# lewisjiang/contour-context

Hardware: AMD Instinct MI355X
Metric: scans/sec ingest+query (120k-pt scan vs 5k-scan DB); max-F1 parity (higher is better)
Workload: dtype f32+f64

## Files before the change

### contour-context_amd/csrc/cc_db_api.inc

```

namespace {

#define CC_ZC_MAX 64
#define CC_NVIEW 4
#define CC_NSTAGE 4
struct ScanLite {
  float keys[CC_NQLEV][CC_NPIV][CC_KEY_DIM];
  int n_cont[CC_HOT_LEVELS];
  int flags;
};

}

#define CC_N_HEADS 24
__global__ void __launch_bounds__(256)
cc_k_pack_hot(const cc_scan_desc_t *__restrict__ desc, int n, cc_hot_desc_t *__restrict__ hot,
              int *__restrict__ z_heads , int *__restrict__ z_pass_cnt ,
              const cc_query_meta *__restrict__ meta_src ,
              cc_query_meta *__restrict__ meta_dst, const int *__restrict__ sel ) {
  const int i = blockIdx.x;
  if (i >= n) return;
  const cc_scan_desc_t *d = desc + (sel ? sel[i] : i);
  cc_hot_desc_t *o = hot + i;
  const int tid = threadIdx.x, nt = blockDim.x;
// ... 486 lines not shown
  if (!db || n < 1 || n > cc_db::NLANE) return set_err(CC_EINVAL, "cc_db_set_lanes: 1 .. 4 lanes");
  {
    const int rc = cc_db_query_wait(db);
    if (rc != CC_OK) return rc;
  }
  HIPCHK(hipSetDevice(db->device));
  for (int i = 0; i < n; i++) {
    const int rc = lane_alloc(db, db->lane[i]);
    if (rc != CC_OK) return rc;
  }
  db->n_lanes = n;
  db->next_lane = 0;
  return CC_OK;
}

int cc_db_size(const cc_db *db) { return db ? db->n_scans : 0; }
int cc_db_knn_stride(const cc_db *db) { return db ? db->kmax : 0; }

void cc_packed_sizes(size_t *hot_bytes, size_t *feat_bytes) {
  if (hot_bytes) *hot_bytes = sizeof(cc_hot_desc_t);
  if (feat_bytes) *feat_bytes = sizeof(cc_gmm_feat);
}
const void *cc_db_hot_ptr(const cc_db *db) { return db ? db->d_hot : nullptr; }
const void *cc_db_feat_ptr(const cc_db *db) { return db ? db->d_feat : nullptr; }

int cc_db_bucket_state(const cc_db *db, int32_t *tree_sizes, float *ranges) {
  if (!db || !tree_sizes || !ranges) return set_err(CC_EINVAL, "cc_db_bucket_state: bad argument");
  for (int l = 0; l < CC_NQLEV; l++) {
    for (int b = 0; b < 6; b++) tree_sizes[l * 6 + b] = (l < db->cfg.n_q_levels) ? (int32_t)db->book[l].b[b].tree.size() : 0;
    for (int b = 0; b < 7; b++) ranges[l * 7 + b] = (l < db->cfg.n_q_levels) ? db->book[l].ranges[b] : 0.f;
  }
  return CC_OK;
}

#define DB_DRAIN(db)                            \
  {                                             \
    const int drc_ = cc_db_query_wait(db);      \
    if (drc_ != CC_OK) return drc_;             \
  }
#define DB_POISON_CHK(db, what) \
  if ((db)->poisoned) return set_err(CC_EHIP, what ": the database handle is in a failed state (an earlier HIP error); destroy it")

int cc_db_set_dynamic_thres(cc_db *db, int on) {
  if (!db || (on != 0 && on != 1)) return set_err(CC_EINVAL, "cc_db_set_dynamic_thres: db must be valid and on 0 or 1");
  DB_POISON_CHK(db, "cc_db_set_dynamic_thres");
  if (on) {
    HIPCHK(hipSetDevice(db->device));
    for (auto &ln : db->lane)
      if (ln.d_qmeta) {
        const int rc = lane_alloc_dyn(ln);
        if (rc != CC_OK) return rc;
      }
  }
  db->dyn_thres = on;
  return CC_OK;
}

static void push_idx_state(cc_db *db) {
  bool all = true;
  for (int l = 0; l < db->cfg.n_q_levels; l++) all = all && db->book[l].fullyIndexed();
  if (all) {
    db->idx_slot.push_back(-1);
    return;
  }
  cc_db::IdxRec r;
  for (int l = 0; l < CC_NQLEV; l++) {
    r.full[l] = (l >= db->cfg.n_q_levels || db->book[l].fullyIndexed()) ? 1 : 0;
    for (int b = 0; b < 6; b++) {
      r.iv[l][2 * b] = l < db->cfg.n_q_levels ? db->book[l].b[b].idx_lo : 0.f;
      r.iv[l][2 * b + 1] = l < db->cfg.n_q_levels ? db->book[l].b[b].idx_hi : 0.f;
    }
  }
  db->idx_slot.push_back((int)db->idx_store.size());
  db->idx_store.push_back(r);
}

int cc_pack_scans(cc_ctx *ctx, const cc_scan_desc_t *d_desc, int n, void *d_hot_out, void *d_feat_out, void *stream_) {
  if (!ctx || !d_desc || n < 0 || !d_hot_out || !d_feat_out) return set_err(CC_EINVAL, "cc_pack_scans: bad argument");
  if (n == 0) return CC_OK;
  hipStream_t stream = (hipStream_t)stream_;
  HIPCHK(hipSetDevice(ctx->device));
  hipLaunchKernelGGL(cc_k_pack_hot, dim3(n), dim3(256), 0, stream, d_desc, n, (cc_hot_desc_t *)d_hot_out, (int *)nullptr, (int *)nullptr,
                     (const cc_query_meta *)nullptr, (cc_query_meta *)nullptr, (const int *)nullptr);
  hipLaunchKernelGGL(cc_k_gmm_prep, dim3(n), dim3(CC_GMM_PREP_BLOCK), 0, stream, d_desc, n, (cc_gmm_feat *)d_feat_out, (const int *)nullptr);
  HIPCHK(hipGetLastError());
  return CC_OK;
}

static int fetch_lite(cc_db *db, const cc_hot_desc_t *d_hot, int n, ScanLite *h_out, hipStream_t stream) {
  if (n <= CC_ZC_MAX) {
    hipLaunchKernelGGL(cc_k_extract, dim3(n), dim3(64), 0, stream, d_hot, n, db->cfg.n_q_levels, db->cfg.q_levels[0], db->cfg.q_levels[1],
                       db->cfg.q_levels[2], db->h_lite_zc);
    HIPCHK(hipGetLastError());
    HIPCHK(hipStreamSynchronize(stream));
    memcpy(h_out, db->h_lite_zc, sizeof(ScanLite) * (size_t)n);
    return CC_OK;
  }
  for (int b0 = 0; b0 < n; b0 += 4096) {
    const int nb = n - b0 < 4096 ? n - b0 : 4096;
    hipLaunchKernelGGL(cc_k_extract, dim3(nb), dim3(64), 0, stream, d_hot + b0, nb, db->cfg.n_q_levels, db->cfg.q_levels[0],
                       db->cfg.q_levels[1], db->cfg.q_levels[2], db->d_lite);
    HIPCHK(hipGetLastError());
    HIPCHK(hipMemcpyAsync(h_out + b0, db->d_lite, sizeof(ScanLite) * nb, hipMemcpyDeviceToHost, stream));
    HIPCHK(hipStreamSynchronize(stream));
  }
  return CC_OK;
}

static int add_settle(cc_db *db) {
  if (db->add_pending) {
    db->add_pending = false;
    HIPCHK(hipEventSynchronize(db->add_done));
  }
  return CC_OK;
}

static int add_scans_device_part(cc_db *db, const int *old_n, const std::vector<int> *ent, const int *act_lo, hipStream_t stream) {
  const int nql = db->cfg.n_q_levels;
  if (db->add_done && db->add_stream != stream) HIPCHK(hipStreamWaitEvent(stream, db->add_done, 0));
  cc_kappend_params AP;
  size_t used = 0;
  size_t need = 0;
  for (int l = 0; l < nql; l++) need += ent[l].size() + (act_lo[l] < db->n_keys[l] ? (size_t)(db->n_keys[l] - act_lo[l]) : 0);
  if (need > db->add_cap) return set_err(CC_ECAPACITY, "cc_db_add_scans: staging buffer too small");
  const bool small_stage = need <= (size_t)CC_ZC_MAX * 64;
  int *h_stage = db->h_add;
  int stage_slot = -1;
  if (small_stage) {
    stage_slot = db->add_small_next;
    db->add_small_next = (stage_slot + 1) % CC_NSTAGE;
    if (db->add_small_busy[stage_slot]) {
      HIPCHK(hipEventSynchronize(db->add_small_ev[stage_slot]));
      db->add_small_busy[stage_slot] = false;
    }
    h_stage = db->h_add_small[stage_slot];
  } else {
    const int src_ = add_settle(db);
    if (src_ != CC_OK) return src_;
  }
  AP.cap_k = db->cap_k;
  for (int l = 0; l < CC_NQLEV; l++) {
    AP.keys[l] = db->d_keys[l];
    AP.kgidx[l] = db->d_kgidx[l];
    AP.kseq[l] = db->d_kseq[l];
    AP.n_old[l] = l < nql ? old_n[l] : 0;
    AP.q_levels[l] = l < nql ? db->cfg.q_levels[l] : 1;
    AP.first[l] = (int)used;
    if (l < nql && !ent[l].empty()) {
      memcpy(h_stage + used, ent[l].data(), sizeof(int) * ent[l].size());
      used += ent[l].size();
    }
  }
  AP.first[CC_NQLEV] = (int)used;
  const size_t n_ent = used;
  size_t act_off[CC_NQLEV] = {0, 0, 0};
  for (int l = 0; l < nql; l++) {
    act_off[l] = used;
    if (act_lo[l] < db->n_keys[l]) {
      const size_t cnt = (size_t)(db->n_keys[l] - act_lo[l]);
      memcpy(h_stage + used, db->book[l].active_from.data() + act_lo[l], sizeof(int) * cnt);
      used += cnt;
    }
  }
  const bool zc = used <= (size_t)CC_ZC_MAX * 64;
  size_t act_total = 0;
  for (int l = 0; l < CC_NQLEV; l++) {
    AP.act_first[l] = (int)act_total;
// ... 151 lines not shown
int cc_db_add_scans(cc_db *db, const cc_scan_desc_t *d_desc, int n, const double *h_ts, const int32_t *h_seed, void *stream_) {
  if (!db || !d_desc || n < 0 || !h_ts || !h_seed) return set_err(CC_EINVAL, "cc_db_add_scans: bad argument");
  DB_POISON_CHK(db, "cc_db_add_scans");
  if (db->n_scans + n > db->cap) return set_err(CC_ECAPACITY, "cc_db_add_scans: database capacity exceeded");
  if (n == 0) return CC_OK;
  hipStream_t stream = (hipStream_t)stream_;
  HIPCHK(hipSetDevice(db->device));
  if (db->prep_cnt > 0) {
    cc_db::Prepared &pp = db->prep[db->prep_head];
    if (pp.d_desc != d_desc || pp.n != n || pp.row0 != db->n_scans)
      return set_err(CC_EINVAL, "cc_db_add_scans: batches prepared with cc_db_add_scans_prepare must be added first, in the order they were prepared");
    HIPCHK(hipStreamWaitEvent(stream, pp.ev, 0));
    HIPCHK(hipEventSynchronize(pp.ev));
    db->prep_head = (db->prep_head + 1) % cc_db::PREP_SLOTS;
    db->prep_cnt--;
    db->n_prepared -= n;
    const int rc_p = add_scans_commit(db, n, h_ts, h_seed, stream, pp.h_lite);
    if (rc_p != CC_OK && db->prep_cnt > 0) {
      cc_db::Prepared &nx = db->prep[db->prep_head];
      hipEventSynchronize(nx.ev);
      db->prep_cnt = 0;
      db->n_prepared = 0;
    }
    return rc_p;
  }
  int rc = cc_pack_scans(db->ctx, d_desc, n, db->d_hot + db->n_scans, db->d_feat + db->n_scans, stream_);
  if (rc != CC_OK) return rc;
  return add_scans_commit(db, n, h_ts, h_seed, stream);
}

int cc_db_add_scans_prepare(cc_db *db, const cc_scan_desc_t *d_desc, int n, void *stream_) {
  if (!db || !d_desc || n < 1 || n > cc_db::PREP_MAX) return set_err(CC_EINVAL, "cc_db_add_scans_prepare: bad argument (1..4096 scans)");
  DB_POISON_CHK(db, "cc_db_add_scans_prepare");
  if (db->prep_cnt >= cc_db::PREP_SLOTS) return set_err(CC_EINVAL, "cc_db_add_scans_prepare: two prepared batches are already waiting to be added");
  if (db->n_scans + db->n_prepared + n > db->cap) return set_err(CC_ECAPACITY, "cc_db_add_scans_prepare: database capacity exceeded");
  hipStream_t stream = (hipStream_t)stream_;
  HIPCHK(hipSetDevice(db->device));
  cc_db::Prepared &pp = db->prep[(db->prep_head + db->prep_cnt) % cc_db::PREP_SLOTS];
  if (!pp.ev) {
    HIPCHK(hipEventCreateWithFlags(&pp.ev, hipEventDisableTiming));
    HIPCHK(hipMalloc(&pp.d_lite, sizeof(ScanLite) * cc_db::PREP_MAX));
    HIPCHK(hipHostMalloc((void **)&pp.h_lite, sizeof(ScanLite) * cc_db::PREP_MAX, hipHostMallocDefault));
  }
  const int row0 = db->n_scans + db->n_prepared;
  int rc = cc_pack_scans(db->ctx, d_desc, n, db->d_hot + row0, db->d_feat + row0, stream_);
  if (rc != CC_OK) return rc;
  hipLaunchKernelGGL(cc_k_extract, dim3(n), dim3(64), 0, stream, (const cc_hot_desc_t *)(db->d_hot + row0), n, db->cfg.n_q_levels,
                     db->cfg.q_levels[0], db->cfg.q_levels[1], db->cfg.q_levels[2], pp.d_lite);
  HIPCHK(hipGetLastError());
  HIPCHK(hipMemcpyAsync(pp.h_lite, pp.d_lite, sizeof(ScanLite) * (size_t)n, hipMemcpyDeviceToHost, stream));
  HIPCHK(hipEventRecord(pp.ev, stream));
  pp.d_desc = d_desc;
  pp.n = n;
  pp.row0 = row0;
  db->prep_cnt++;
  db->n_prepared += n;
  return CC_OK;
}

int cc_db_add_packed(cc_db *db, const void *d_hot, const void *d_feat, int n, const double *h_ts, const int32_t *h_seed, void *stream_) {
  if (!db || !d_hot || !d_feat || n < 0 || !h_ts || !h_seed) return set_err(CC_EINVAL, "cc_db_add_packed: bad argument");
  DB_POISON_CHK(db, "cc_db_add_packed");
  if (db->prep_cnt > 0) return set_err(CC_EINVAL, "cc_db_add_packed: batches prepared with cc_db_add_scans_prepare are waiting to be added");
  if (db->n_scans + n > db->cap) return set_err(CC_ECAPACITY, "cc_db_add_packed: database capacity exceeded");
  if (n == 0) return CC_OK;
  hipStream_t stream = (hipStream_t)stream_;
  HIPCHK(hipSetDevice(db->device));
  HIPCHK(hipMemcpyAsync(db->d_hot + db->n_scans, d_hot, sizeof(cc_hot_desc_t) * (size_t)n, hipMemcpyDeviceToDevice, stream));
  HIPCHK(hipMemcpyAsync(db->d_feat + db->n_scans, d_feat, sizeof(cc_gmm_feat) * (size_t)n, hipMemcpyDeviceToDevice, stream));
  return add_scans_commit(db, n, h_ts, h_seed, stream);
}

static bool thres_strict_smaller(const cc_score_t *lb, const cc_score_t *ub) {
  return lb->i_ovlp_sum < ub->i_ovlp_sum && lb->i_ovlp_max_one < ub->i_ovlp_max_one && lb->i_in_ang_rng < ub->i_in_ang_rng &&
         lb->i_indiv_sim < ub->i_indiv_sim && lb->i_orie_sim < ub->i_orie_sim && lb->correlation < ub->correlation &&
         lb->area_perc < ub->area_perc && lb->neg_est_dist < ub->neg_est_dist;
}

static int launch_query_prep(cc_db *db, cc_qlane &ln, const cc_scan_desc_t *d_q, int nb, bool meta_from_host = false, const int *d_sel = nullptr) {
  (void)db;
  hipStream_t ls = ln.stream;
  hipLaunchKernelGGL(cc_k_pack_hot, dim3(nb), dim3(256), 0, ls, d_q, nb, ln.d_qhot, ln.d_heads, ln.d_pass_cnt,
                     meta_from_host ? (const cc_query_meta *)ln.h_meta : (const cc_query_meta *)nullptr, ln.d_qmeta, d_sel);
  hipLaunchKernelGGL(cc_k_gmm_prep, dim3(nb), dim3(CC_GMM_PREP_BLOCK), 0, ls, d_q, nb, ln.d_qfeat, d_sel);
  HIPCHK(hipGetLastError());
  return CC_OK;
}

static int launch_scoring_chain(cc_db *db, cc_qlane &ln, int nb, const cc_check_params &CP, const cc_score_t *lb, const cc_score_t *ub,
                                int max_fine_opt, hipEvent_t *ev, int *d_scores, bool zc ,
                                int km) {
  hipStream_t ls = ln.stream;
  const bool lg = km != CC_KNN_MAX;
  const bool dyn = db->dyn_thres != 0;
  if (dyn && !ln.d_tidy) return set_err(CC_EHIP, "launch_scoring_chain: the lane has no dynamic-threshold buffers");
  cc_pass_rec *const dpass = dyn ? ln.d_pass : nullptr;
  unsigned char *const dok = dyn ? ln.d_pass_ok : nullptr;
  const cc_hot_desc_t *qh = ln.d_qhot, *dh = db->d_hot;
  const size_t n_slots = (size_t)nb * CC_CHK_STRIDE_K(km);
  hipLaunchKernelGGL(lg ? cc_k_check_a_l : cc_k_check_a, dim3((unsigned)((n_slots + CC_CHKA_BLOCK - 1) / CC_CHKA_BLOCK)), dim3(CC_CHKA_BLOCK), 0, ls, CP, qh, dh, nb, (const cc_knn_hit_t *)ln.d_hits,
                     (const int *)ln.d_hit_cnt, ln.d_items, ln.d_cnt, ln.d_pass_ok, ln.d_pass_cnt, d_scores, dpass);
  hipLaunchKernelGGL((lg ? cc_k_check_b1_l<CC_PP_SMALL, false> : cc_k_check_b1<CC_PP_SMALL, false>), dim3(db->tune.b1), dim3(64), 0, ls, CP, qh, dh, (const cc_chk_item *)ln.d_items,
                     ln.d_redo, ln.d_cnt, ln.d_cstl, ln.d_pass_cnt, d_scores, dpass, dok);
  hipLaunchKernelGGL((lg ? cc_k_check_b1_l<CC_PP_MAX, true> : cc_k_check_b1<CC_PP_MAX, true>), dim3((db->tune.b1 + 3) / 4), dim3(64), 0, ls, CP, qh, dh, (const cc_chk_item *)ln.d_items, ln.d_redo,
                     ln.d_cnt, ln.d_cstl, ln.d_pass_cnt, d_scores, dpass, dok);
  hipLaunchKernelGGL(cc_k_compact_cstl, dim3((unsigned)((n_slots + CC_CHKA_BLOCK - 1) / CC_CHKA_BLOCK)), dim3(CC_CHKA_BLOCK), 0, ls, CP, (const cc_cstl_item *)ln.d_cstl, ln.d_cnt,
                     ln.d_cstl_idx);
  hipLaunchKernelGGL(lg ? cc_k_check_b2_l : cc_k_check_b2, dim3(db->tune.b2), dim3(64), 0, ls, CP, qh, dh, (const cc_cstl_item *)ln.d_cstl,
                     (const int *)ln.d_cstl_idx, (const int *)ln.d_cnt, ln.d_pass, ln.d_pass_ok, ln.d_pass_cnt, d_scores, dyn ? 1 : 0);
  hipLaunchKernelGGL(lg ? cc_k_check_c_l : cc_k_check_c, dim3((db->tune.b2 + 3) / 4), dim3(256), 0, ls, (const cc_cstl_item *)ln.d_cstl,
                     (const int *)ln.d_cstl_idx, (const int *)ln.d_cnt, ln.d_pass, (const unsigned char *)ln.d_pass_ok);
  if (dyn)
    hipLaunchKernelGGL(lg ? cc_k_check_dyn_l : cc_k_check_dyn, dim3(nb), dim3(64), 0, ls, nb, *lb, *ub, (const cc_pass_rec *)ln.d_pass, ln.d_pass_ok, ln.d_pass_cnt,
                       d_scores);
  if (ev) HIPCHK(hipEventRecord(ev[2], ls));
  hipLaunchKernelGGL(lg ? cc_k_merge_l : cc_k_merge, dim3(nb), dim3(CC_MERGE_BLOCK), 0, ls, nb, *lb, db->n_row, db->n_col, qh, dh, (const cc_pass_rec *)ln.d_pass,
                     (const unsigned char *)ln.d_pass_ok, (const int *)ln.d_pass_cnt, ln.d_cands, ln.d_qstate, ln.d_prob, ln.d_prob_list,
                     ln.d_nprob, dyn ? ln.d_cpost : (cc_cand_post *)nullptr);
  if (ev) HIPCHK(hipEventRecord(ev[3], ls));
  hipLaunchKernelGGL(cc_k_gmm_init, dim3(db->tune.gmm), dim3(64), 0, ls, (const cc_gmm_problem *)ln.d_prob, (const int *)ln.d_prob_list,
                     (const int *)ln.d_nprob, (const cc_gmm_feat *)ln.d_qfeat, (const cc_gmm_feat *)db->d_feat, ln.d_gres,
                     cc_gmm_code_pool{ln.d_codes, ln.code_cap, ln.d_heads + 9, ln.d_nprob + 3, ln.pool_cap});
  hipLaunchKernelGGL(lg ? (dyn ? cc_k_select_l<true> : cc_k_select_l<false>) : (dyn ? cc_k_select<true> : cc_k_select<false>), dim3(nb), dim3(64), 0, ls, nb, lb->correlation, max_fine_opt,
                     (const cc_cand_out *)ln.d_cands, (const cc_qstate *)ln.d_qstate, (const cc_gmm_result *)ln.d_gres, ln.d_sel, ln.prob_cap,
                     ln.d_nprob + 1, ln.d_heads + 8, (const unsigned short *)db->d_perm_tab, ln.d_sel + 3 * (size_t)ln.prob_cap, ln.d_heads + 12,
                     ln.d_nprob + 3, ln.d_pool_off, (const cc_cand_post *)ln.d_cpost, ln.d_tidy, *lb, *ub);
  hipLaunchKernelGGL(cc_k_gmm_refine<16>, dim3(db->tune.gmm), dim3(64), 0, ls, (const cc_gmm_problem *)ln.d_prob, (const int *)(ln.d_nprob + 1),
                     (const int *)ln.d_sel, (const int *)(ln.d_heads + 8), (const int *)(ln.d_sel + 2 * (size_t)ln.prob_cap), (const int *)(ln.d_nprob + 2),
                     (const cc_gmm_feat *)ln.d_qfeat, (const cc_gmm_feat *)db->d_feat, lb->correlation, ln.d_pool,
                     ln.pool_cap, (const int *)ln.d_pool_off, ln.d_gres, (const unsigned *)ln.d_codes, (const int *)nullptr, (const int *)nullptr, 0);
  hipLaunchKernelGGL(cc_k_gmm_refine<64>, dim3(db->tune.gmm64), dim3(64), 0, ls, (const cc_gmm_problem *)ln.d_prob, (const int *)(ln.d_nprob + 2),
                     (const int *)(ln.d_sel + ln.prob_cap), (const int *)(ln.d_heads + 8), (const int *)(ln.d_sel + 2 * (size_t)ln.prob_cap),
                     (const int *)(ln.d_nprob + 1), (const cc_gmm_feat *)ln.d_qfeat, (const cc_gmm_feat *)db->d_feat, lb->correlation,
                     ln.d_pool, ln.pool_cap, (const int *)ln.d_pool_off, ln.d_gres, (const unsigned *)ln.d_codes,
                     (const int *)(ln.d_sel + 3 * (size_t)ln.prob_cap), (const int *)(ln.d_heads + 12), ln.prob_cap);
  if (ev) HIPCHK(hipEventRecord(ev[4], ls));
  hipLaunchKernelGGL(lg ? (dyn ? cc_k_final_l<true> : cc_k_final_l<false>) : (dyn ? cc_k_final<true> : cc_k_final<false>), dim3(nb), dim3(64), 0, ls, nb, lb->correlation, max_fine_opt,
                     (const cc_cand_out *)ln.d_cands, (const cc_qstate *)ln.d_qstate, (const cc_gmm_result *)ln.d_gres, (const int *)ln.d_pass_cnt,
                     (const int *)ln.d_hit_cnt, qh, zc ? ln.h_results : ln.d_results, (const unsigned short *)db->d_perm_tab, (const int *)ln.d_nprob,
                     zc ? ln.h_nprob : (int *)nullptr, (const unsigned char *)ln.d_tidy);
  if (ev) HIPCHK(hipEventRecord(ev[5], ls));
  HIPCHK(hipGetLastError());
  return CC_OK;
}

static int chunk_status(const cc_qlane &ln, int nb) {
  if (ln.h_nprob[3] > ln.pool_cap) return set_err(CC_ECAPACITY, "the pair pool (or the pair-code pool) of the correlation refinement overflowed");
  for (int i = 0; i < nb; i++)
    if (ln.h_results[i].flags)
      return set_err(CC_ECAPACITY, "a query met an internal capacity of the scoring kernels (cc_query_result_t.flags, CC_QF_*): "
                                   "its result may differ from the reference's");
  return CC_OK;
}

static int lane_finish(cc_db *db, cc_qlane &ln) {
  if (!ln.busy) return CC_OK;
  ln.busy = false;
  HIPCHK(hipStreamSynchronize(ln.stream));
  memcpy(ln.h_dst + ln.b0, ln.h_results, sizeof(cc_query_result_t) * ln.nb);
  if (ln.profiled) {
    float t[5];
    for (int k = 0; k < 5; k++) hipEventElapsedTime(&t[k], ln.pev[k], ln.pev[k + 1]);
    const double w = (double)ln.nb;
    for (int k = 0; k < 5; k++) db->ms_acc[k] += t[k];
    db->launch_w += w;
  }
  return chunk_status(ln, ln.nb);
}

static void lane_abort(cc_db *db, cc_qlane &ln) {
  if (ln.stream) {
    hipStreamCaptureStatus cs = hipStreamCaptureStatusNone;
    if (hipStreamIsCapturing(ln.stream, &cs) == hipSuccess && cs != hipStreamCaptureStatusNone) {
      hipGraph_t g = nullptr;
      if (hipStreamEndCapture(ln.stream, &g) == hipSuccess && g) hipGraphDestroy(g);
      (void)hipGetLastError();
    }
  }
  if (ln.stream) hipStreamSynchronize(ln.stream);
  ln.busy = false;
  db->poisoned = true;
}

int cc_db_query_wait(cc_db *db) {
  if (!db) return set_err(CC_EINVAL, "cc_db_query_wait: bad argument");
  HIPCHK(hipSetDevice(db->device));
  int rc = CC_OK;
  for (auto &ln : db->lane) {
    const int r2 = lane_finish(db, ln);
    if (rc == CC_OK) rc = r2;
  }
  return rc;
}

int cc_db_query_collect(cc_db *db, const cc_query_result_t *h_res, int n) {
  if (!db || !h_res || n < 1) return set_err(CC_EINVAL, "cc_db_query_collect: bad argument");
  HIPCHK(hipSetDevice(db->device));
  int rc = CC_OK;
  for (auto &ln : db->lane) {
    if (!ln.busy) continue;
    const cc_query_result_t *lo = ln.h_dst + ln.b0, *hi = lo + ln.nb;
    if (hi <= h_res || lo >= h_res + n) continue;
// ... 551 lines not shown
```

### contour-context_amd/csrc/k_gmm.h

```cpp
#pragma once
#include "cc_dev.h"
#include "cc_group.h"
#include "cc_sort.h"
#include "cc_fmath.h"
#include "k_merge.h"

#define CC_GMM_ECAP_L CC_MAXC
#ifndef CC_GMM_G16_MAX_PAIRS
#define CC_GMM_G16_MAX_PAIRS 96
#endif
#ifndef CC_GMM_MID_MAX_PAIRS
#define CC_GMM_MID_MAX_PAIRS 256
#endif
#ifndef CC_GMM_PACK_MIN_PROBLEMS
#define CC_GMM_PACK_MIN_PROBLEMS 3072
#endif

#define CC_GMM_NCLS 8
#ifndef CC_GMM_WPE
#define CC_GMM_WPE 2
#endif
__device__ __forceinline__ int cc_gmm_len_class(int np) {
  return np > 1400 ? 0 : (np > 1100 ? 1 : (np > 950 ? 2 : (np > 850 ? 3 : (np > 750 ? 4 : (np > 650 ? 5 : (np > 500 ? 6 : 7))))));
}

struct cc_gmm_result {
  double corr_init;
  double corr_opt;
  double tf_opt[3];
  int optimized;
  int iterations;
  int termination;
  int flags;
  int n_pairs;
  int code_seg;
};

struct cc_ell {
  float c00, c01, c10, c11, mx, my, w, maj;
};

struct cc_gmm_feat {
  int n_ell[CC_GMM_LEVELS];
  int flags;
  int pad[3];
  double ac;
  cc_ell ell[CC_GMM_LEVELS][CC_GMM_ECAP_L];
};

__device__ __forceinline__ double cc_gmm_self_term(const cc_ell &a, const cc_ell &b) {
  const double n00 = 2.0 * ((double)a.c00 + (double)b.c00), n01 = 2.0 * ((double)a.c01 + (double)b.c01);
  const double n10 = 2.0 * ((double)a.c10 + (double)b.c10), n11 = 2.0 * ((double)a.c11 + (double)b.c11);
  const double mx = (double)a.mx - (double)b.mx, my = (double)a.my - (double)b.my;
  const double det = n00 * n11 - n10 * n01, invdet = 1.0 / det;
  const double i00 = n11 * invdet, i10 = -n10 * invdet, i01 = -n01 * invdet, i11 = n00 * invdet;
  const double h0 = -0.5 * mx, h1 = -0.5 * my;
  const double r0 = h0 * i00 + h1 * i10, r1 = h0 * i01 + h1 * i11;
  return (double)a.w * (double)b.w / sqrt(det) * exp(r0 * mx + r1 * my);
}

#define CC_GMM_PREP_BLOCK 256
__global__ void __launch_bounds__(CC_GMM_PREP_BLOCK)
cc_k_gmm_prep(const cc_scan_desc_t *__restrict__ desc, int n, cc_gmm_feat *__restrict__ feat,
              const int *__restrict__ sel ) {
  const int tid = threadIdx.x, lane = tid & 63, wave = tid >> 6;
  constexpr int NW = CC_GMM_PREP_BLOCK / 64;
  if ((int)blockIdx.x >= n) return;
  const cc_scan_desc_t *d = desc + (sel ? sel[blockIdx.x] : (int)blockIdx.x);
  cc_gmm_feat *F = feat + blockIdx.x;
  __shared__ cc_ell E[CC_GMM_ECAP_L];
  __shared__ unsigned s_q[NW][128];
  __shared__ double s_part[NW];
  int flags = 0;
  double acc = 0;
  for (int li = 0; li < CC_GMM_LEVELS; li++) {
    const int lev = li + 1;
    const int full = d->layer_cell_cnt[lev];
    const int ncont = d->n_cont[lev], nst = d->n_stored[lev];
    int n_use = 0, run = 0;
    for (int j0 = 0; j0 < ncont; j0 += 64) {
      const int j = j0 + lane;
      const int cnt = (j < ncont && j < nst) ? d->cont[lev][j].cell_cnt : 0;
      int incl = cnt;
      for (int o = 1; o < 64; o <<= 1) {
        const int v = __shfl_up(incl, o);
        if (lane >= o) incl += v;
      }
      const int before = run + incl - cnt;
      const bool use = j < ncont && !((double)before * 1.0 / (double)full >= 0.95);
      const unsigned long long m = __ballot(use);
      if (__ballot(use && j >= nst)) flags |= 4;
      n_use += __popcll(m);
      run += __shfl(incl, 63);
      if (m != ~0ull) break;
    }
    if (n_use > nst) n_use = nst;
    if (n_use > CC_GMM_ECAP_L) {
      n_use = CC_GMM_ECAP_L;
      flags |= 1;
    }
    __syncthreads();
    for (int j = tid; j < n_use; j += CC_GMM_PREP_BLOCK) {
      const cc_contour_t &cv = d->cont[lev][j];
      const float v00 = cv.eig_vecs[0], v10 = cv.eig_vecs[1], v01 = cv.eig_vecs[2], v11 = cv.eig_vecs[3];
      const float e0 = cv.eig_vals[0], e1 = cv.eig_vals[1];
      const float a00 = v00 * e0, a01 = v01 * e1, a10 = v10 * e0, a11 = v11 * e1;
      cc_ell e;
      e.c00 = a00 * v00 + a01 * v01;
      e.c01 = a00 * v10 + a01 * v11;
      e.c10 = a10 * v00 + a11 * v01;
      e.c11 = a10 * v10 + a11 * v11;
      e.mx = cv.pos_mean[0];
      e.my = cv.pos_mean[1];
      e.w = (float)cv.cell_cnt;
      e.maj = sqrtf(e1);
      E[j] = e;
      F->ell[li][j] = e;
    }
    __syncthreads();
    const int nrow = (n_use + 1) >> 1, wid = n_use + 1, tot = nrow * wid;
    int qh = 0, qn = 0;
    for (int i0 = wave * 64; i0 < tot; i0 += CC_GMM_PREP_BLOCK) {
      const int idx = i0 + lane;
      bool go = false;
      int i = 0, j = 0;
      if (idx < tot) {
        const int r = idx / wid, c = idx - r * wid;
        if (c < n_use - r) {
          i = r;
          j = r + c;
          go = true;
        } else if (n_use - 1 - r != r) {
          i = n_use - 1 - r;
          j = i + (c - (n_use - r));
          go = true;
        }
      }
      if (go) {
        const cc_ell a = E[i], b = E[j];
        const float dx = a.mx - b.mx, dy = a.my - b.my;
        const float t00 = a.c00 + b.c00, t11 = a.c11 + b.c11, t01 = a.c01 + b.c01, t10 = a.c10 + b.c10;
        const float tr = t00 + t11, det = t00 * t11 - t01 * t10;
        if (dx * dx + dy * dy > 400.f * tr && det > 1e-4f * tr * tr) go = false;
      }
      const unsigned long long m = __ballot(go);
      if (go) s_q[wave][(qh + qn + __popcll(m & ((1ull << lane) - 1ull))) & 127] = ((unsigned)i << 16) | (unsigned)j;
      qn += __popcll(m);
      cc_wave_sync();
      if (qn >= 64) {
        const unsigned e = s_q[wave][(qh + lane) & 127];
        const int ei = (int)(e >> 16), ej = (int)(e & 0xFFFFu);
        const double t = cc_gmm_self_term(E[ei], E[ej]);
        acc += ei == ej ? t : 2.0 * t;
        qh = (qh + 64) & 127;
        qn -= 64;
        cc_wave_sync();
      }
    }
    if (lane < qn) {
      const unsigned e = s_q[wave][(qh + lane) & 127];
      const int ei = (int)(e >> 16), ej = (int)(e & 0xFFFFu);
      const double t = cc_gmm_self_term(E[ei], E[ej]);
      acc += ei == ej ? t : 2.0 * t;
    }
    cc_wave_sync();
    if (tid == 0) F->n_ell[li] = n_use;
  }
  for (int o = 32; o > 0; o >>= 1) acc += __shfl_xor(acc, o);
  if (lane == 0) s_part[wave] = acc;
  __syncthreads();
  if (tid == 0) {
    double t = 0;
    for (int w = 0; w < NW; w++) t += s_part[w];
    F->ac = t;
    F->flags = flags;
  }
}


struct cc_gpair {
  double sd, sb;
  double a00, a11;
  double as, ap;
  double w;
  double pad_;
  float smx, smy, tmx, tmy;
};
static_assert(sizeof(cc_gpair) == 80, "the pose-independent half of a term, in registers");
struct cc_graw {
  float4 s;
  float4 t;
  float4 m;
  float2 w;
};
#define CC_GRAW_BYTES 56
#ifndef CC_GMM_NL
#define CC_GMM_NL 128
#endif
struct cc_gsrc {
  float4 *lds;
  char *glb;
  int nl_cap, nl, ng_alloc;
};
__device__ __forceinline__ cc_graw cc_gsrc_load(const cc_gsrc &Q, int i) {
  cc_graw r;
  if (i < Q.nl) {
    r.s = Q.lds[i];
    r.t = Q.lds[Q.nl_cap + i];
    r.m = Q.lds[2 * Q.nl_cap + i];
    r.w = ((const float2 *)(Q.lds + 3 * Q.nl_cap))[i];
  } else {
    const int j = i - Q.nl;
    const float4 *g = (const float4 *)Q.glb + j;
    r.s = g[0];
    r.t = g[Q.ng_alloc];
    r.m = g[2 * (size_t)Q.ng_alloc];
    r.w = ((const float2 *)((const float4 *)Q.glb + 3 * (size_t)Q.ng_alloc))[j];
  }
  return r;
}
__device__ __forceinline__ void cc_gsrc_store(const cc_gsrc &Q, int i, const cc_graw &r) {
  if (i < Q.nl) {
    Q.lds[i] = r.s;
    Q.lds[Q.nl_cap + i] = r.t;
    Q.lds[2 * Q.nl_cap + i] = r.m;
    ((float2 *)(Q.lds + 3 * Q.nl_cap))[i] = r.w;
  } else {
    const int j = i - Q.nl;
    float4 *g = (float4 *)Q.glb + j;
    g[0] = r.s;
    g[Q.ng_alloc] = r.t;
    g[2 * (size_t)Q.ng_alloc] = r.m;
    ((float2 *)((float4 *)Q.glb + 3 * (size_t)Q.ng_alloc))[j] = r.w;
  }
}

template <int G>
__device__ __forceinline__ double cc_gsum(double v) {
  if (G >= 64) {
    v += __shfl_xor(v, 32);
    v += __shfl_xor(v, 16);
  }
  return cc_group_sum_d(v);
}
template <int G>
__device__ __forceinline__ void cc_gsum4(double &a, double &b, double &c, double &d) {
  a = cc_gsum<G>(a);
  b = cc_gsum<G>(b);
  c = cc_gsum<G>(c);
  d = cc_gsum<G>(d);
}

struct cc_gterm {
  double v, gx, gy, gt;
};
__device__ __forceinline__ cc_gterm cc_gmm_term(const cc_gpair &P, double px, double py, double c, double s, double c2, double s2,
                                                const double *exp_tab) {
  const double p = fma(P.sd, c2, -(P.sb * s2)), q = fma(P.sd, s2, P.sb * c2);
  const double p2 = p + p, q2 = q + q;
// ... 1330 lines not shown
```

### contour-context_amd/csrc/k_merge.h

```cpp
#pragma once
#include "cc_dev.h"
#include "k_check.h"

#define CC_MAXCAND CC_CHK_STRIDE
#define CC_MERGE_BLOCK 64

struct cc_gmm_problem {
  int q;
  int gidx;
  double tf[3];
};

struct cc_dprop {
  unsigned long long bits[7];
  double c, s, tx, ty;
  double ang;
  int vote_cnt;
  float area_perc;
};
struct cc_dcand {
  int gidx, nprops, gmm_idx, pad;
  cc_dprop props[4];
};
struct cc_cand_out {
  int gidx, nprops, gmm_idx, pad;
};
struct cc_cand_post {
  double neg_est_dist;
  float area_perc;
  int pad;
};
struct cc_qstate {
  int n_cand;
  int flags;
};
template <int STR>
struct alignas(16) cc_merge_lds {
  cc_dcand st[CC_MERGE_BLOCK];
  alignas(16) int gid[STR];
  unsigned short ord[STR];
  short next[STR];
  unsigned short firstrec[STR];
  alignas(16) int cg[STR + 4];
  unsigned short clast[STR];
  int base;
  unsigned char want[STR];
  float tperc[CC_HOT_LEVELS][CC_NDIST];
};

static_assert(CC_CHK_STRIDE % CC_MERGE_BLOCK == 0 && CC_CHK_STRIDE_K(CC_KNN_MAX_LARGE) % CC_MERGE_BLOCK == 0, "merge scan split");
static_assert(CC_CHK_STRIDE_K(CC_KNN_MAX_LARGE) <= 32767, "check slots and list positions are kept in u16 / short");
static_assert(CC_MERGE_BLOCK == 64, "the list building below uses wave ballots");

template <int KM>
__device__ __forceinline__ void cc_merge_body(int nq, cc_score_t lb, int n_row, int n_col, const cc_hot_desc_t *qdesc,
                                              const cc_hot_desc_t *db_desc, const cc_pass_rec *pass, const unsigned char *pass_ok,
                                              const int *pass_cnt, cc_cand_out *cands_all, cc_qstate *qstate,
                                              cc_gmm_problem *probs ,
                                              int *prob_list , int *n_prob,
                                              cc_cand_post *post ) {
  __shared__ cc_merge_lds<CC_CHK_STRIDE_K(KM)> L;
  const int q = blockIdx.x, tid = threadIdx.x, lane = tid & 63;
  if (q >= nq) return;
  const unsigned char *okp = pass_ok + (size_t)q * CC_CHK_STRIDE_K(KM);
  const cc_pass_rec *recs = pass + (size_t)q * CC_CHK_STRIDE_K(KM);
  const unsigned long long lt_mask = (1ull << lane) - 1ull;
  if (tid < CC_HOT_LEVELS * CC_NDIST) {
    const int l = tid / CC_NDIST, t_ = tid - l * CC_NDIST;
    const cc_hot_desc_t *tq = qdesc + q;
    L.tperc[l][t_] = (float)tq->cont[l][t_].cell_cnt * 1.0f / (float)tq->layer_cell_cnt[l];
  }
  int n = 0;
  constexpr int NU = CC_CHK_STRIDE / 64;
  for (int u0 = 0; u0 < CC_CHK_STRIDE_K(KM) / 64; u0 += NU) {
    unsigned char okv[NU];
#pragma unroll
    for (int u = 0; u < NU; u++) okv[u] = okp[(u0 + u) * 64 + lane];
#pragma unroll
    for (int u = 0; u < NU; u++) {
      const bool ok = okv[u] != 0;
      const unsigned long long m = __ballot(ok);
      if (ok) L.ord[n + __popcll(m & lt_mask)] = (unsigned short)((u0 + u) * 64 + lane);
      n += __popcll(m);
    }
  }
  __syncthreads();
  for (int i0 = 0; i0 < n; i0 += 4 * CC_MERGE_BLOCK) {
    int g[4];
#pragma unroll
    for (int u = 0; u < 4; u++) {
      const int i = i0 + u * CC_MERGE_BLOCK + lane;
      g[u] = i < n ? recs[L.ord[i]].gidx : 0;
    }
#pragma unroll
    for (int u = 0; u < 4; u++) {
      const int i = i0 + u * CC_MERGE_BLOCK + lane;
      if (i < n) {
        L.gid[i] = g[u];
        L.next[i] = -1;
      }
    }
  }
  __syncthreads();
  int nc = 0;
  if (lane < 4) L.cg[lane] = -1;
  __syncthreads();
  for (int b0 = 0; b0 < n; b0 += CC_MERGE_BLOCK) {
    const int i = b0 + lane;
    const bool valid = i < n;
    const int g = valid ? L.gid[i] : 0;
    int k = -1;
    for (int j0 = 0; j0 < nc; j0 += 4) {
      const int4 v = *(const int4 *)&L.cg[j0];
      k = v.x == g ? j0 : (v.y == g ? j0 + 1 : (v.z == g ? j0 + 2 : (v.w == g ? j0 + 3 : k)));
    }
    if (!valid) k = -1;
    const int before = k >= 0 ? (int)L.clast[k] : -1;
    unsigned long long rem = __ballot(valid);
    int prev_lane = -1, lead_lane = lane;
    bool last_in_round = false;
    while (rem) {
      const int lead = __ffsll(rem) - 1;
      const int g_lead = __builtin_amdgcn_readlane(g, lead);
      const bool mine = valid && g == g_lead;
      const unsigned long long same = __ballot(mine);
      if (mine) {
        const unsigned long long lower = same & lt_mask;
        prev_lane = lower ? 63 - __builtin_clzll(lower) : -1;
        lead_lane = lead;
        last_in_round = (same >> lane) == 1ull;
      }
      rem &= ~same;
    }
    const bool opens = valid && k < 0 && prev_lane < 0;
    const unsigned long long mo = __ballot(opens);
    int kk = k;
    if (opens) {
      kk = nc + __popcll(mo & lt_mask);
      L.cg[kk] = g;
      L.firstrec[kk] = (unsigned short)i;
    }
    const int k_lead = __shfl(kk, lead_lane);
    if (valid && kk < 0) kk = k_lead;
    if (valid) {
      if (prev_lane >= 0)
        L.next[b0 + prev_lane] = (short)i;
      else if (before >= 0)
        L.next[before] = (short)i;
      if (last_in_round) L.clast[kk] = (unsigned short)i;
    }
    nc += __popcll(mo);
    if (lane < 4) L.cg[nc + lane] = -1;
    __syncthreads();
  }
  __syncthreads();
  if (tid == 0) {
    cc_qstate st;
    st.n_cand = nc;
    st.flags = 0;
    qstate[q] = st;
  }
  cc_dcand *c = &L.st[tid];
  for (int k = tid; k < nc; k += CC_MERGE_BLOCK) {
    int i = L.firstrec[k];
    c->gidx = L.gid[i];
    c->nprops = 0;
    const cc_pass_rec *rec = &recs[L.ord[i]];
    int np_n = rec->n_pairs;
    double ptx_n = rec->tf[0], pty_n = rec->tf[1], pc_n = rec->cs[0], ps_n = rec->cs[1], ang_n = rec->cs[2];
    for (; i >= 0;) {
      rec = &recs[L.ord[i]];
      const int np = np_n;
      const double ptx = ptx_n, pty = pty_n;
      const double pc = pc_n, ps = ps_n, ang2_cur = ang_n;
      i = L.next[i];
      if (i >= 0) {
        const cc_pass_rec *rn = &recs[L.ord[i]];
        np_n = rn->n_pairs;
        ptx_n = rn->tf[0];
        pty_n = rn->tf[1];
        pc_n = rn->cs[0];
        ps_n = rn->cs[1];
        ang_n = rn->cs[2];
      }
      const int nprops = c->nprops;
      int hit = -1;
      for (int pi = 0; pi < nprops && hit < 0; pi++) {
        const cc_dprop *p = &c->props[pi];
        const double i00 = pc, i01 = ps, i10 = -ps, i11 = pc;
        const double itx = -(i00 * ptx + i01 * pty), ity = -(i10 * ptx + i11 * pty);
        const double d00 = i00 * p->c + i01 * p->s, d10 = i10 * p->c + i11 * p->s;
        const double dtx = i00 * p->tx + i01 * p->ty + itx, dty = i10 * p->tx + i11 * p->ty + ity;
        const double n2 = dtx * dtx + dty * dty;
        bool near_t = n2 < 4.0 * (1.0 - 1e-9);
        if (!near_t && n2 <= 4.0 * (1.0 + 1e-9)) near_t = sqrt(n2) < 2.0;
        if (near_t) {
          const double t03 = 0.30933624960962325;
          const double ay = fabs(d10), lim = d00 * t03;
          bool near_r = d00 > 0.0 && ay < lim * (1.0 - 1e-9);
          if (!near_r && d00 > 0.0 && ay <= lim * (1.0 + 1e-9)) near_r = fabs(atan2(d10, d00)) < 0.3;
          if (near_r) hit = pi;
        }
      }
      if (hit >= 0) {
        cc_dprop *p = &c->props[hit];
        for (int w = 0; w < 7; w++) p->bits[w] |= rec->bits[w];
        p->vote_cnt += np;
        const int w1 = p->vote_cnt, w2 = np;
        const double bx = (p->tx * w1 + ptx * w2) / (w1 + w2), by = (p->ty * w1 + pty * w2) / (w1 + w2);
        const double ang1 = p->ang, ang2 = ang2_cur;
        double diff = ang2 - ang1;
        if (diff < 0) diff += 2 * 3.14159265358979323846;
        if (diff > 3.14159265358979323846) diff -= 2 * 3.14159265358979323846;
        const double ang_bl = diff * w2 / (w1 + w2) + ang1;
        double sn, cs;
        sincos(ang_bl, &sn, &cs);
        p->c = cs;
        p->s = sn;
        double aw = ang_bl;
        if (aw > 3.14159265358979323846) aw -= 2 * 3.14159265358979323846;
        if (aw <= -3.14159265358979323846) aw += 2 * 3.14159265358979323846;
        p->ang = aw;
        p->tx = bx;
        p->ty = by;
      } else if (nprops <= 3) {
        cc_dprop *p = &c->props[nprops];
        for (int w = 0; w < 7; w++) p->bits[w] = rec->bits[w];
        p->c = pc;
        p->s = ps;
        p->ang = ang2_cur;
        p->tx = ptx;
        p->ty = pty;
        p->vote_cnt = np;
        p->area_perc = 0.f;
        c->nprops = nprops + 1;
      }
    }
    const cc_hot_desc_t *sl = db_desc + c->gidx;
    int idx_sel = 0;
    for (int pi = 0; pi < c->nprops; pi++) {
      float lev_perc[CC_NLEV] = {0, 0, 0, 0, 0, 0};
      for (int w = 0; w < 7; w++) {
        unsigned long long m = c->props[pi].bits[w];
        while (m) {
          const int b = w * 64 + (__ffsll((unsigned long long)m) - 1);
          m &= m - 1;
          const int l = b / 100 + 1, s_ = (b % 100) / 10, t_ = b % 10;
          const float psrc = (float)sl->cont[l - 1][s_].cell_cnt * 1.0f / (float)sl->layer_cell_cnt[l - 1];
          const float ptgt = L.tperc[l - 1][t_];
          lev_perc[l] += 0.5f * (psrc + ptgt);
        }
      }
      float perc = 0.f;
      perc += 0.3f * lev_perc[1];
      perc += 0.3f * lev_perc[2];
      perc += 0.3f * lev_perc[3];
      perc += 0.1f * lev_perc[4];
      c->props[pi].area_perc = perc;
      if (c->props[pi].vote_cnt > c->props[idx_sel].vote_cnt) idx_sel = pi;
    }
    const cc_dprop *p0 = &c->props[idx_sel];
    int gi = -1;
    if (!(p0->area_perc < lb.area_perc)) {
      const double ox = n_row / 2 - 0.5, oy = n_col / 2 - 0.5;
      const double mx = p0->c * ox + (-p0->s) * oy + p0->tx, my = p0->s * ox + p0->c * oy + p0->ty;
      const double ex = 1.0 * mx + 0.0 * my + (-(1.0 * ox + 0.0 * oy)), ey = 0.0 * mx + 1.0 * my + (-(0.0 * ox + 1.0 * oy));
      const double neg = -sqrt(ex * ex + ey * ey);
      if (!(neg < (double)lb.neg_est_dist)) {
        gi = q * CC_CHK_STRIDE_K(KM) + k;
        cc_gmm_problem pb;
        pb.q = q;
        pb.gidx = c->gidx;
        pb.tf[0] = p0->tx;
        pb.tf[1] = p0->ty;
        pb.tf[2] = p0->ang;
        probs[gi] = pb;
        if (post) {
          cc_cand_post cp;
          cp.neg_est_dist = neg;
          cp.area_perc = p0->area_perc;
          cp.pad = 0;
          post[gi] = cp;
        }
      }
    }
    L.want[k] = gi >= 0 ? 1 : 0;
    cc_cand_out o;
    o.gidx = c->gidx;
    o.nprops = c->nprops;
    o.gmm_idx = gi;
    o.pad = 0;
    cands_all[(size_t)q * CC_CHK_STRIDE_K(KM) + k] = o;
  }
  __syncthreads();
  int n_want = 0;
  for (int b0 = 0; b0 < nc; b0 += CC_MERGE_BLOCK) {
    const int k = b0 + tid;
    const bool w = k < nc && L.want[k];
    const unsigned long long m = __ballot(w);
    if (w) L.ord[n_want + __popcll(m & lt_mask)] = (unsigned short)k;
    n_want += __popcll(m);
  }
  if (tid == 0) L.base = n_want ? atomicAdd(n_prob, n_want) : 0;
  __syncthreads();
  for (int i = tid; i < n_want; i += CC_MERGE_BLOCK) prob_list[L.base + i] = q * CC_CHK_STRIDE_K(KM) + (int)L.ord[i];
}

__global__ void __launch_bounds__(CC_MERGE_BLOCK)
cc_k_merge(int nq, cc_score_t lb, int n_row, int n_col, const cc_hot_desc_t *__restrict__ qdesc,
           const cc_hot_desc_t *__restrict__ db_desc, const cc_pass_rec *__restrict__ pass, const unsigned char *__restrict__ pass_ok,
           const int *__restrict__ pass_cnt, cc_cand_out *__restrict__ cands_all, cc_qstate *__restrict__ qstate,
           cc_gmm_problem *__restrict__ probs ,
           int *__restrict__ prob_list , int *__restrict__ n_prob,
           cc_cand_post *__restrict__ post ) {
  cc_merge_body<CC_KNN_MAX>(nq, lb, n_row, n_col, qdesc, db_desc, pass, pass_ok, pass_cnt, cands_all, qstate, probs, prob_list, n_prob, post);
}
__global__ void __launch_bounds__(CC_MERGE_BLOCK)
cc_k_merge_l(int nq, cc_score_t lb, int n_row, int n_col, const cc_hot_desc_t *__restrict__ qdesc,
             const cc_hot_desc_t *__restrict__ db_desc, const cc_pass_rec *__restrict__ pass, const unsigned char *__restrict__ pass_ok,
             const int *__restrict__ pass_cnt, cc_cand_out *__restrict__ cands_all, cc_qstate *__restrict__ qstate,
             cc_gmm_problem *__restrict__ probs ,
             int *__restrict__ prob_list , int *__restrict__ n_prob,
             cc_cand_post *__restrict__ post ) {
  cc_merge_body<CC_KNN_MAX_LARGE>(nq, lb, n_row, n_col, qdesc, db_desc, pass, pass_ok, pass_cnt, cands_all, qstate, probs, prob_list, n_prob, post);
}
```

Before: 603,000.

## Defer query GMM self-sum until after merge and skip queries without problems

Splits the GMM prep kernel into an ellipse-building pass, run at query prep, and a self-correlation sum pass that runs after merge. The second pass reads each query's problem count, newly recorded by merge, and exits early for queries that own no correlation problem. This avoids the quadratic pairwise self-term work for queries that never reach GMM scoring. In exchange it adds an extra kernel launch, reloads the ellipses from global memory, and removes the sel parameter from the DB-side prep kernel.

```diff
diff --git a/contour-context_amd/csrc/cc_db_api.inc b/contour-context_amd/csrc/cc_db_api.inc
--- a/contour-context_amd/csrc/cc_db_api.inc
+++ b/contour-context_amd/csrc/cc_db_api.inc
@@ -592,7 +592,7 @@
   HIPCHK(hipSetDevice(ctx->device));
   hipLaunchKernelGGL(cc_k_pack_hot, dim3(n), dim3(256), 0, stream, d_desc, n, (cc_hot_desc_t *)d_hot_out, (int *)nullptr, (int *)nullptr,
                      (const cc_query_meta *)nullptr, (cc_query_meta *)nullptr, (const int *)nullptr);
-  hipLaunchKernelGGL(cc_k_gmm_prep, dim3(n), dim3(CC_GMM_PREP_BLOCK), 0, stream, d_desc, n, (cc_gmm_feat *)d_feat_out, (const int *)nullptr);
+  hipLaunchKernelGGL(cc_k_gmm_prep, dim3(n), dim3(CC_GMM_PREP_BLOCK), 0, stream, d_desc, n, (cc_gmm_feat *)d_feat_out);
   HIPCHK(hipGetLastError());
   return CC_OK;
 }
@@ -910,7 +910,7 @@
   hipStream_t ls = ln.stream;
   hipLaunchKernelGGL(cc_k_pack_hot, dim3(nb), dim3(256), 0, ls, d_q, nb, ln.d_qhot, ln.d_heads, ln.d_pass_cnt,
                      meta_from_host ? (const cc_query_meta *)ln.h_meta : (const cc_query_meta *)nullptr, ln.d_qmeta, d_sel);
-  hipLaunchKernelGGL(cc_k_gmm_prep, dim3(nb), dim3(CC_GMM_PREP_BLOCK), 0, ls, d_q, nb, ln.d_qfeat, d_sel);
+  hipLaunchKernelGGL(cc_k_gmm_prep_ell, dim3(nb), dim3(CC_GMM_PREP_BLOCK), 0, ls, d_q, nb, ln.d_qfeat, d_sel);
   HIPCHK(hipGetLastError());
   return CC_OK;
 }
@@ -946,6 +946,7 @@
                      (const unsigned char *)ln.d_pass_ok, (const int *)ln.d_pass_cnt, ln.d_cands, ln.d_qstate, ln.d_prob, ln.d_prob_list,
                      ln.d_nprob, dyn ? ln.d_cpost : (cc_cand_post *)nullptr);
   if (ev) HIPCHK(hipEventRecord(ev[3], ls));
+  hipLaunchKernelGGL(cc_k_gmm_prep_ac, dim3(nb), dim3(CC_GMM_PREP_BLOCK), 0, ls, nb, ln.d_qfeat, (const cc_qstate *)ln.d_qstate);
   hipLaunchKernelGGL(cc_k_gmm_init, dim3(db->tune.gmm), dim3(64), 0, ls, (const cc_gmm_problem *)ln.d_prob, (const int *)ln.d_prob_list,
                      (const int *)ln.d_nprob, (const cc_gmm_feat *)ln.d_qfeat, (const cc_gmm_feat *)db->d_feat, ln.d_gres,
                      cc_gmm_code_pool{ln.d_codes, ln.code_cap, ln.d_heads + 9, ln.d_nprob + 3, ln.pool_cap});
diff --git a/contour-context_amd/csrc/k_gmm.h b/contour-context_amd/csrc/k_gmm.h
--- a/contour-context_amd/csrc/k_gmm.h
+++ b/contour-context_amd/csrc/k_gmm.h
@@ -60,13 +60,124 @@
 }
 
 #define CC_GMM_PREP_BLOCK 256
+
+template <bool TO_LDS>
+__device__ __forceinline__ int cc_gmm_prep_ellipses(const cc_scan_desc_t *__restrict__ d, int li, cc_gmm_feat *__restrict__ F, cc_ell *E,
+                                                    int &flags) {
+  const int tid = threadIdx.x, lane = tid & 63;
+  const int lev = li + 1;
+  const int full = d->layer_cell_cnt[lev];
+  const int ncont = d->n_cont[lev], nst = d->n_stored[lev];
+  int n_use = 0, run = 0;
+  for (int j0 = 0; j0 < ncont; j0 += 64) {
+    const int j = j0 + lane;
+    const int cnt = (j < ncont && j < nst) ? d->cont[lev][j].cell_cnt : 0;
+    int incl = cnt;
+    for (int o = 1; o < 64; o <<= 1) {
+      const int v = __shfl_up(incl, o);
+      if (lane >= o) incl += v;
+    }
+    const int before = run + incl - cnt;
+    const bool use = j < ncont && !((double)before * 1.0 / (double)full >= 0.95);
+    const unsigned long long m = __ballot(use);
+    if (__ballot(use && j >= nst)) flags |= 4;
+    n_use += __popcll(m);
+    run += __shfl(incl, 63);
+    if (m != ~0ull) break;
+  }
+  if (n_use > nst) n_use = nst;
+  if (n_use > CC_GMM_ECAP_L) {
+    n_use = CC_GMM_ECAP_L;
+    flags |= 1;
+  }
+  if (TO_LDS) __syncthreads();
+  for (int j = tid; j < n_use; j += CC_GMM_PREP_BLOCK) {
+    const cc_contour_t &cv = d->cont[lev][j];
+    const float v00 = cv.eig_vecs[0], v10 = cv.eig_vecs[1], v01 = cv.eig_vecs[2], v11 = cv.eig_vecs[3];
+    const float e0 = cv.eig_vals[0], e1 = cv.eig_vals[1];
+    const float a00 = v00 * e0, a01 = v01 * e1, a10 = v10 * e0, a11 = v11 * e1;
+    cc_ell e;
+    e.c00 = a00 * v00 + a01 * v01;
+    e.c01 = a00 * v10 + a01 * v11;
+    e.c10 = a10 * v00 + a11 * v01;
+    e.c11 = a10 * v10 + a11 * v11;
+    e.mx = cv.pos_mean[0];
+    e.my = cv.pos_mean[1];
+    e.w = (float)cv.cell_cnt;
+    e.maj = sqrtf(e1);
+    if (TO_LDS) E[j] = e;
+    F->ell[li][j] = e;
+  }
+  return n_use;
+}
+
+__device__ __forceinline__ void cc_gmm_prep_self_sum(const cc_ell *E, int n_use, unsigned *s_q, double &acc) {
+  const int tid = threadIdx.x, lane = tid & 63, wave = tid >> 6;
+  const int nrow = (n_use + 1) >> 1, wid = n_use + 1, tot = nrow * wid;
+  int qh = 0, qn = 0;
+  for (int i0 = wave * 64; i0 < tot; i0 += CC_GMM_PREP_BLOCK) {
+    const int idx = i0 + lane;
+    bool go = false;
+    int i = 0, j = 0;
+    if (idx < tot) {
+      const int r = idx / wid, c = idx - r * wid;
+      if (c < n_use - r) {
+        i = r;
+        j = r + c;
+        go = true;
+      } else if (n_use - 1 - r != r) {
+        i = n_use - 1 - r;
+        j = i + (c - (n_use - r));
+        go = true;
+      }
+    }
+    if (go) {
+      const cc_ell a = E[i], b = E[j];
+      const float dx = a.mx - b.mx, dy = a.my - b.my;
+      const float t00 = a.c00 + b.c00, t11 = a.c11 + b.c11, t01 = a.c01 + b.c01, t10 = a.c10 + b.c10;
+      const float tr = t00 + t11, det = t00 * t11 - t01 * t10;
+      if (dx * dx + dy * dy > 400.f * tr && det > 1e-4f * tr * tr) go = false;
+    }
+    const unsigned long long m = __ballot(go);
+    if (go) s_q[(qh + qn + __popcll(m & ((1ull << lane) - 1ull))) & 127] = ((unsigned)i << 16) | (unsigned)j;
+    qn += __popcll(m);
+    cc_wave_sync();
+    if (qn >= 64) {
+      const unsigned e = s_q[(qh + lane) & 127];
+      const int ei = (int)(e >> 16), ej = (int)(e & 0xFFFFu);
+      const double t = cc_gmm_self_term(E[ei], E[ej]);
+      acc += ei == ej ? t : 2.0 * t;
+      qh = (qh + 64) & 127;
+      qn -= 64;
+      cc_wave_sync();
+    }
+  }
+  if (lane < qn) {
+    const unsigned e = s_q[(qh + lane) & 127];
+    const int ei = (int)(e >> 16), ej = (int)(e & 0xFFFFu);
+    const double t = cc_gmm_self_term(E[ei], E[ej]);
+    acc += ei == ej ? t : 2.0 * t;
+  }
+  cc_wave_sync();
+}
+
+__device__ __forceinline__ double cc_gmm_prep_reduce(double acc, double *s_part) {
+  const int tid = threadIdx.x, lane = tid & 63, wave = tid >> 6;
+  for (int o = 32; o > 0; o >>= 1) acc += __shfl_xor(acc, o);
+  if (lane == 0) s_part[wave] = acc;
+  __syncthreads();
+  double t = 0;
+  if (tid == 0)
+    for (int w = 0; w < CC_GMM_PREP_BLOCK / 64; w++) t += s_part[w];
+  return t;
+}
+
 __global__ void __launch_bounds__(CC_GMM_PREP_BLOCK)
-cc_k_gmm_prep(const cc_scan_desc_t *__restrict__ desc, int n, cc_gmm_feat *__restrict__ feat,
-              const int *__restrict__ sel ) {
-  const int tid = threadIdx.x, lane = tid & 63, wave = tid >> 6;
+cc_k_gmm_prep(const cc_scan_desc_t *__restrict__ desc, int n, cc_gmm_feat *__restrict__ feat) {
+  const int tid = threadIdx.x, wave = tid >> 6;
   constexpr int NW = CC_GMM_PREP_BLOCK / 64;
   if ((int)blockIdx.x >= n) return;
-  const cc_scan_desc_t *d = desc + (sel ? sel[blockIdx.x] : (int)blockIdx.x);
+  const cc_scan_desc_t *d = desc + blockIdx.x;
   cc_gmm_feat *F = feat + blockIdx.x;
   __shared__ cc_ell E[CC_GMM_ECAP_L];
   __shared__ unsigned s_q[NW][128];
@@ -74,107 +185,51 @@
   int flags = 0;
   double acc = 0;
   for (int li = 0; li < CC_GMM_LEVELS; li++) {
-    const int lev = li + 1;
-    const int full = d->layer_cell_cnt[lev];
-    const int ncont = d->n_cont[lev], nst = d->n_stored[lev];
-    int n_use = 0, run = 0;
-    for (int j0 = 0; j0 < ncont; j0 += 64) {
-      const int j = j0 + lane;
-      const int cnt = (j < ncont && j < nst) ? d->cont[lev][j].cell_cnt : 0;
-      int incl = cnt;
-      for (int o = 1; o < 64; o <<= 1) {
-        const int v = __shfl_up(incl, o);
-        if (lane >= o) incl += v;
-      }
-      const int before = run + incl - cnt;
-      const bool use = j < ncont && !((double)before * 1.0 / (double)full >= 0.95);
-      const unsigned long long m = __ballot(use);
-      if (__ballot(use && j >= nst)) flags |= 4;
-      n_use += __popcll(m);
-      run += __shfl(incl, 63);
-      if (m != ~0ull) break;
-    }
-    if (n_use > nst) n_use = nst;
-    if (n_use > CC_GMM_ECAP_L) {
-      n_use = CC_GMM_ECAP_L;
-      flags |= 1;
-    }
+    const int n_use = cc_gmm_prep_ellipses<true>(d, li, F, E, flags);
     __syncthreads();
-    for (int j = tid; j < n_use; j += CC_GMM_PREP_BLOCK) {
-      const cc_contour_t &cv = d->cont[lev][j];
-      const float v00 = cv.eig_vecs[0], v10 = cv.eig_vecs[1], v01 = cv.eig_vecs[2], v11 = cv.eig_vecs[3];
-      const float e0 = cv.eig_vals[0], e1 = cv.eig_vals[1];
-      const float a00 = v00 * e0, a01 = v01 * e1, a10 = v10 * e0, a11 = v11 * e1;
-      cc_ell e;
-      e.c00 = a00 * v00 + a01 * v01;
-      e.c01 = a00 * v10 + a01 * v11;
-      e.c10 = a10 * v00 + a11 * v01;
-      e.c11 = a10 * v10 + a11 * v11;
-      e.mx = cv.pos_mean[0];
-      e.my = cv.pos_mean[1];
-      e.w = (float)cv.cell_cnt;
-      e.maj = sqrtf(e1);
-      E[j] = e;
-      F->ell[li][j] = e;
-    }
-    __syncthreads();
-    const int nrow = (n_use + 1) >> 1, wid = n_use + 1, tot = nrow * wid;
-    int qh = 0, qn = 0;
-    for (int i0 = wave * 64; i0 < tot; i0 += CC_GMM_PREP_BLOCK) {
-      const int idx = i0 + lane;
-      bool go = false;
-      int i = 0, j = 0;
-      if (idx < tot) {
-        const int r = idx / wid, c = idx - r * wid;
-        if (c < n_use - r) {
-          i = r;
-          j = r + c;
-          go = true;
-        } else if (n_use - 1 - r != r) {
-          i = n_use - 1 - r;
-          j = i + (c - (n_use - r));
-          go = true;
-        }
-      }
-      if (go) {
-        const cc_ell a = E[i], b = E[j];
-        const float dx = a.mx - b.mx, dy = a.my - b.my;
-        const float t00 = a.c00 + b.c00, t11 = a.c11 + b.c11, t01 = a.c01 + b.c01, t10 = a.c10 + b.c10;
-        const float tr = t00 + t11, det = t00 * t11 - t01 * t10;
-        if (dx * dx + dy * dy > 400.f * tr && det > 1e-4f * tr * tr) go = false;
-      }
-      const unsigned long long m = __ballot(go);
-      if (go) s_q[wave][(qh + qn + __popcll(m & ((1ull << lane) - 1ull))) & 127] = ((unsigned)i << 16) | (unsigned)j;
-      qn += __popcll(m);
-      cc_wave_sync();
-      if (qn >= 64) {
-        const unsigned e = s_q[wave][(qh + lane) & 127];
-        const int ei = (int)(e >> 16), ej = (int)(e & 0xFFFFu);
-        const double t = cc_gmm_self_term(E[ei], E[ej]);
-        acc += ei == ej ? t : 2.0 * t;
-        qh = (qh + 64) & 127;
-        qn -= 64;
-        cc_wave_sync();
-      }
-    }
-    if (lane < qn) {
-      const unsigned e = s_q[wave][(qh + lane) & 127];
-      const int ei = (int)(e >> 16), ej = (int)(e & 0xFFFFu);
-      const double t = cc_gmm_self_term(E[ei], E[ej]);
-      acc += ei == ej ? t : 2.0 * t;
-    }
-    cc_wave_sync();
+    cc_gmm_prep_self_sum(E, n_use, s_q[wave], acc);
     if (tid == 0) F->n_ell[li] = n_use;
   }
-  for (int o = 32; o > 0; o >>= 1) acc += __shfl_xor(acc, o);
-  if (lane == 0) s_part[wave] = acc;
-  __syncthreads();
+  const double t = cc_gmm_prep_reduce(acc, s_part);
   if (tid == 0) {
-    double t = 0;
-    for (int w = 0; w < NW; w++) t += s_part[w];
     F->ac = t;
     F->flags = flags;
   }
+}
+
+__global__ void __launch_bounds__(CC_GMM_PREP_BLOCK)
+cc_k_gmm_prep_ell(const cc_scan_desc_t *__restrict__ desc, int n, cc_gmm_feat *__restrict__ feat,
+                  const int *__restrict__ sel ) {
+  if ((int)blockIdx.x >= n) return;
+  const cc_scan_desc_t *d = desc + (sel ? sel[blockIdx.x] : (int)blockIdx.x);
+  cc_gmm_feat *F = feat + blockIdx.x;
+  int flags = 0;
+  for (int li = 0; li < CC_GMM_LEVELS; li++) {
+    const int n_use = cc_gmm_prep_ellipses<false>(d, li, F, nullptr, flags);
+    if (threadIdx.x == 0) F->n_ell[li] = n_use;
+  }
+  if (threadIdx.x == 0) F->flags = flags;
+}
+
+__global__ void __launch_bounds__(CC_GMM_PREP_BLOCK)
+cc_k_gmm_prep_ac(int n, cc_gmm_feat *__restrict__ feat, const cc_qstate *__restrict__ qstate) {
+  const int tid = threadIdx.x, wave = tid >> 6;
+  constexpr int NW = CC_GMM_PREP_BLOCK / 64;
+  if ((int)blockIdx.x >= n || qstate[blockIdx.x].n_prob == 0) return;
+  cc_gmm_feat *F = feat + blockIdx.x;
+  __shared__ cc_ell E[CC_GMM_ECAP_L];
+  __shared__ unsigned s_q[NW][128];
+  __shared__ double s_part[NW];
+  double acc = 0;
+  for (int li = 0; li < CC_GMM_LEVELS; li++) {
+    const int n_use = F->n_ell[li];
+    __syncthreads();
+    for (int j = tid; j < n_use; j += CC_GMM_PREP_BLOCK) E[j] = F->ell[li][j];
+    __syncthreads();
+    cc_gmm_prep_self_sum(E, n_use, s_q[wave], acc);
+  }
+  const double t = cc_gmm_prep_reduce(acc, s_part);
+  if (tid == 0) F->ac = t;
 }
 
 
diff --git a/contour-context_amd/csrc/k_merge.h b/contour-context_amd/csrc/k_merge.h
--- a/contour-context_amd/csrc/k_merge.h
+++ b/contour-context_amd/csrc/k_merge.h
@@ -33,6 +33,7 @@
 struct cc_qstate {
   int n_cand;
   int flags;
+  int n_prob;
 };
 template <int STR>
 struct alignas(16) cc_merge_lds {
@@ -158,6 +159,7 @@
     cc_qstate st;
     st.n_cand = nc;
     st.flags = 0;
+    st.n_prob = 0;
     qstate[q] = st;
   }
   cc_dcand *c = &L.st[tid];
@@ -301,7 +303,10 @@
     if (w) L.ord[n_want + __popcll(m & lt_mask)] = (unsigned short)k;
     n_want += __popcll(m);
   }
-  if (tid == 0) L.base = n_want ? atomicAdd(n_prob, n_want) : 0;
+  if (tid == 0) {
+    L.base = n_want ? atomicAdd(n_prob, n_want) : 0;
+    qstate[q].n_prob = n_want;
+  }
   __syncthreads();
   for (int i = tid; i < n_want; i += CC_MERGE_BLOCK) prob_list[L.base + i] = q * CC_CHK_STRIDE_K(KM) + (int)L.ord[i];
 }
diff --git a/profiles/lazy_query_prep/trace_summary.py b/profiles/lazy_query_prep/trace_summary.py
--- /dev/null
+++ b/profiles/lazy_query_prep/trace_summary.py
@@ -0,0 +1,40 @@
+import collections
+import csv
+import re
+import sys
+
+rows = list(csv.DictReader(open(sys.argv[1])))
+steps = int(sys.argv[2])
+
+
+def name(r):
+    return re.sub(r"\(.*", "", r["Kernel_Name"]).replace("void ", "").strip()
+
+
+tot, cnt = collections.Counter(), collections.Counter()
+for r in rows:
+    tot[name(r)] += int(r["End_Timestamp"]) - int(r["Start_Timestamp"])
+    cnt[name(r)] += 1
+print("%-44s %8s %14s   (whole run: set-up appends and the isolated steps included; per step = / %d)" % ("kernel", "launches", "us per step", steps))
+for k, v in sorted(tot.items(), key=lambda kv: -kv[1]):
+    if k.startswith("cc_k_") or k.startswith("cc_"):
+        print("%-44s %8d %14.1f" % (k[:44], cnt[k], v / 1e3 / steps))
+by_q = collections.defaultdict(list)
+for r in rows:
+    by_q[(r.get("Agent_Id"), r.get("Queue_Id"))].append(r)
+pred = collections.Counter()
+for q, rs in by_q.items():
+    rs.sort(key=lambda r: int(r["Start_Timestamp"]))
+    for a, b in zip(rs, rs[1:]):
+        if name(b).startswith("cc_k_gmm_prep"):
+            pred[(name(b), name(a))] += 1
+print("\nlaunch in front of it on the same queue:")
+for (b, a), n in sorted(pred.items()):
+    print("  %-20s <- %-28s x %d" % (b, a[:28], n))
+if len(sys.argv) > 3:
+    import os
+    import numpy as np
+    pose = np.load(os.path.join(sys.argv[3], "query_n_cand_pose.npy"))
+    tidy = np.load(os.path.join(sys.argv[3], "query_n_cand_tidy.npy"))
+    print("\nqueries of the last timed step that own no correlation problem: between %.3f (no candidate at all: %d of %d) and %.3f "
+          "(no candidate after the correlation bar)" % ((pose == 0).mean(), (pose == 0).sum(), pose.size, (tidy == 0).mean()))
```

Result: slower. 581,000 (-3.7%).
